# ExistentialRobotics/CORSAIR

Hardware: AMD Instinct MI355X
Metric: end-to-end queries/sec (embed+retrieve+register), Scan2CAD chair (higher is better)
Workload: dtype f32 sparse conv + embedding / f64 RANSAC, k-NN, Chamfer, top-k / f16 MFMA bounds and shortlists (survivors recounted in f64)

## Files before the change

corsair_amd/csrc/hardneg.hip:

```cpp
#include <hipcub/hipcub.hpp>

#include "nn_common.h"

namespace cs {

struct HnProb {
  int64_t t0;
  int32_t tn;
  int32_t pad;
};

struct HnTile {
  int32_t a0;
  int32_t an;
  int32_t prob;
  int32_t pad;
};

constexpr int HN_NG = 2;
constexpr int HN_QT = 4 * 32 * HN_NG;
constexpr int HN_KK = 4;
constexpr int32_t HN_NONE = 0x7fffffff;
constexpr int HN_EX_GRID = 4096;

// ... 47 lines not shown
}

__global__ void k_hn_pack_targets(const float* __restrict__ tf, int ld, const float* __restrict__ txyz,
                                  const int64_t* __restrict__ toff, _Float16* __restrict__ img,
                                  float4* __restrict__ t4, unsigned* __restrict__ seg_t2max_bits) {
  const int sg = blockIdx.y;
  const int64_t b = toff[sg], e = toff[sg + 1];
  float mx = 0.f;
  for (int64_t j = b + blockIdx.x * (int64_t)blockDim.x + threadIdx.x; j < e; j += (int64_t)gridDim.x * blockDim.x) {
    const double n2 = knf_pack_target_row(tf + j * ld, img + j * KNF_PITCH);
    t4[j] = make_float4(txyz[3 * j], txyz[3 * j + 1], txyz[3 * j + 2], (float)n2);
    mx = fmaxf(mx, (float)n2 * 1.0000002f);
  }
  knf_seg_max(mx, &seg_t2max_bits[sg]);
}

__global__ void k_hn_pack_anchors(const float* __restrict__ qf, int ld, const float* __restrict__ qxyz,
                                  const int32_t* __restrict__ anchor, const uint32_t* __restrict__ keys_sorted,
                                  const int32_t* __restrict__ vals_sorted, int64_t A, int n_prob,
                                  _Float16* __restrict__ qrows, float4* __restrict__ q4) {
  const int64_t i = blockIdx.x * (int64_t)blockDim.x + threadIdx.x;
  if (i >= A || keys_sorted[i] >= (uint32_t)n_prob) return;
  const int64_t r = anchor[vals_sorted[i]];
  knf_pack_query_row(qf + r * ld, qrows + i * 48);
  q4[i] = make_float4(qxyz[3 * r], qxyz[3 * r + 1], qxyz[3 * r + 2], 0.f);
}

__global__ __launch_bounds__(256) void k_hn_f16(const HnTile* __restrict__ tiles, const HnProb* __restrict__ probs,
                                                const _Float16* __restrict__ qrows, const float4* __restrict__ q4,
                                                const _Float16* __restrict__ img, const float4* __restrict__ t4,
                                                double r2, int use_excl, int32_t* __restrict__ cand_i,
                                                float* __restrict__ cand_tau) {
  constexpr int STAGE_BYTES = KNF_STAGE_BYTES;
  __shared__ __attribute__((aligned(1024))) char lds[2 * STAGE_BYTES];
  __shared__ __attribute__((aligned(16))) float tn_s[2][KNF_ROWS];
  __shared__ __attribute__((aligned(16))) float4 x_s[2][KNF_ROWS];
  const HnTile tile = tiles[blockIdx.x];
  if (tile.an == 0) return;
  const HnProb pb = probs[tile.prob];
  const int tid = threadIdx.x;
  const int lane = tid & 63;
  const int wave = __builtin_amdgcn_readfirstlane(tid >> 6);
  const int half = lane >> 5;
  const int col = lane & 31;
  f16x8 bop[HN_NG][3];
  double qx[HN_NG], qy[HN_NG], qz[HN_NG];
  bool qvalid[HN_NG];
  float bd[HN_NG][HN_KK], thr[HN_NG];
  int32_t bi[HN_NG][HN_KK];
#pragma unroll
  for (int g = 0; g < HN_NG; ++g) {
    const int qloc = wave * 32 * HN_NG + 32 * g + col;
    qvalid[g] = qloc < tile.an;
    const int64_t qpos = tile.a0 + (qvalid[g] ? qloc : 0);
    const _Float16* row = qrows + qpos * 48 + 8 * half;
#pragma unroll
    for (int m = 0; m < 3; ++m) bop[g][m] = *reinterpret_cast<const f16x8*>(row + 16 * m);
    const float4 p = q4[qpos];
    qx[g] = (double)p.x;
    qy[g] = (double)p.y;
    qz[g] = (double)p.z;
    thr[g] = INFINITY;
#pragma unroll
    for (int j = 0; j < HN_KK; ++j) {
      bd[g][j] = INFINITY;
      bi[g][j] = HN_NONE;
    }
  }
  const int t_hi = pb.tn;
  if (t_hi > 0) {
    const char* gimg = reinterpret_cast<const char*>(img + pb.t0 * KNF_PITCH) + lane * 16;
    const unsigned lds_base = __builtin_amdgcn_readfirstlane(lds_addr_of(lds));
    auto issue_dma = [&](int b, int base) { knf_issue_dma(gimg, lds_base, wave, b, base); };
    auto load_rows = [&](int base, float4& v) {
      int r = base + (tid % KNF_ROWS);
      r = r > t_hi - 1 ? t_hi - 1 : r;
      v = t4[pb.t0 + r];
    };
    auto store_rows = [&](int b, int base, const float4& v) {
      if (tid < KNF_ROWS) {
        tn_s[b][tid] = base + tid < t_hi ? v.w : INFINITY;
        x_s[b][tid] = v;
      }
    };
    {
      float4 v0;
      load_rows(0, v0);
      issue_dma(0, 0);
      store_rows(0, 0, v0);
    }
    int buf = 0;
    for (int base = 0; base < t_hi; base += KNF_ROWS) {
      asm volatile("s_waitcnt vmcnt(0)" ::: "memory");
      __syncthreads();
      const bool more = base + KNF_ROWS < t_hi;
      float4 v_next;
      load_rows(base + KNF_ROWS, v_next);
      if (more) issue_dma(buf ^ 1, base + KNF_ROWS);
#pragma unroll 1
      for (int t = 0; t < KNF_ROWS / 32; ++t) {
        if (base + 32 * t >= t_hi) break;
        f16x8 a[3];
        f32x16 c16;
        knf_load_tile(lds + buf * STAGE_BYTES, tn_s[buf], t, col, half, a, c16);
#pragma unroll
        for (int g = 0; g < HN_NG; ++g) {
          f32x16 d = __builtin_amdgcn_mfma_f32_32x32x16_f16(a[0], bop[g][0], c16, 0, 0, 0);
          d = knf_mfma_lo(a, bop[g], d);
#pragma unroll
          for (int r = 0; r < 16; ++r) {
            const bool hit = d[r] < thr[g];
            if (__any(hit)) {
              if (hit) {
                const int srow = knf_result_row(t, half, r);
                bool adm = true;
                if (use_excl) {
                  const float4 p = x_s[buf][srow];
                  const double dx = qx[g] - (double)p.x, dy = qy[g] - (double)p.y, dz = qz[g] - (double)p.z;
                  adm = !(((dx * dx + dy * dy) + dz * dz) < r2);
                }
                if (adm) knf_insert(bd[g], bi[g], d[r], base + srow);
              }
              thr[g] = fminf(thr[g], knf_pair_min(bd[g][HN_KK - 1]));
            }
          }
// ... 218 lines not shown
  while ((1LL << end_bit) <= (int64_t)n_prob) ++end_bit;
  size_t tmp_bytes = 0;
  CS_HIP_CHECK(hipcub::DeviceRadixSort::SortPairs(nullptr, tmp_bytes, keys.p, keys_sorted.p, vals.p, vals_sorted.p,
                                                  (int)A, 0, end_bit, s));
  CS_REQUIRE(tmp.alloc(tmp_bytes ? tmp_bytes : 1), CS_ERR_HIP, "cs_hardest_negatives: scratch allocation failed");
  CS_HIP_CHECK(hipcub::DeviceRadixSort::SortPairs(tmp.p, tmp_bytes, keys.p, keys_sorted.p, vals.p, vals_sorted.p, (int)A,
                                                  0, end_bit, s));

  if (!use_f16) {
    hipLaunchKernelGGL(k_hn_exhaustive, ex_grid, dim3(256), 0, s, d_qf, ld_q, d_qxyz, d_tf, ld_t, d_txyz, C,
                       d_anchor, keys_sorted.p, vals_sorted.p, A, n_prob, dprobs.p, r2, use_excl, (const int32_t*)nullptr,
                       d_idx, d_dist);
    CS_LAUNCH_CHECK();
    if (stats) {
      g_hn_stats[0] += (unsigned long long)A;
      g_hn_stats[1] += (unsigned long long)A;
    }
    return CS_OK;
  }

  const unsigned n_tile = (unsigned)(ceil_div(A, HN_QT) + n_prob);
  PoolBuf<HnTile> tiles((size_t)n_tile);
  PoolBuf<int32_t> pstart((size_t)n_prob + 1), cand((size_t)A * 2 * HN_KK), flag((size_t)A);
  PoolBuf<_Float16> qrows((size_t)A * 48), img((size_t)(nt_rows + KNF_ROWS) * KNF_PITCH);
  PoolBuf<float4> q4((size_t)A), t4((size_t)(nt_rows ? nt_rows : 1));
  PoolBuf<float> tau((size_t)A);
  PoolBuf<unsigned> t2max((size_t)ntseg);
  PoolBuf<int64_t> dtoff;
  CS_REQUIRE(tiles.p && pstart.p && cand.p && flag.p && qrows.p && img.p && q4.p && t4.p && tau.p && t2max.p, CS_ERR_HIP,
             "cs_hardest_negatives: scratch allocation failed");
  std::vector<int64_t> toff(h_toff, h_toff + ntseg + 1);
  rc = upload(dtoff, toff, s);
  if (rc) return rc;
  CS_HIP_CHECK(hipMemsetAsync(tiles.p, 0, sizeof(HnTile) * n_tile, s));
  CS_HIP_CHECK(hipMemsetAsync(t2max.p, 0, sizeof(unsigned) * ntseg, s));
  CS_HIP_CHECK(hipMemsetAsync(flag.p, 0, sizeof(int32_t) * (size_t)A, s));
  hipLaunchKernelGGL(k_hn_tiles, dim3(1), dim3(256), 0, s, keys_sorted.p, A, n_prob, pstart.p, tiles.p);
  CS_LAUNCH_CHECK();
  if (nt_rows) {
    hipLaunchKernelGGL(k_hn_pack_targets, dim3(16, (unsigned)ntseg), dim3(256), 0, s, d_tf, ld_t, d_txyz, dtoff.p, img.p,
                       t4.p, t2max.p);
    CS_LAUNCH_CHECK();
  }
  hipLaunchKernelGGL(k_hn_pack_anchors, dim3((unsigned)ceil_div(A, 256)), dim3(256), 0, s, d_qf, ld_q, d_qxyz, d_anchor,
                     keys_sorted.p, vals_sorted.p, A, n_prob, qrows.p, q4.p);
  CS_LAUNCH_CHECK();
  hipLaunchKernelGGL(k_hn_f16, dim3(n_tile), dim3(256), 0, s, tiles.p, dprobs.p, qrows.p, q4.p, img.p, t4.p, r2, use_excl,
// ... 21 lines not shown
```

corsair_amd/csrc/knn.hip:

```cpp
#include <hipcub/hipcub.hpp>


#include "nn_common.h"

namespace cs {

struct KnnWork {
  int64_t q0;
  int64_t t0;
  int64_t o0;
  int32_t qn;
  int32_t tn;
  int32_t prob;
  int32_t pad;
};

constexpr int KNN_MAXK = 8;
constexpr int KNN_TT = 128;

template <int DIM>
__global__ __launch_bounds__(256) void k_knn_feat(const KnnWork* __restrict__ work,
                                                  const float* __restrict__ qf,
                                                  const float* __restrict__ tf, int k,
                                                  const int32_t* __restrict__ qlabel,
// ... 68 lines not shown
    for (int j = 0; j < k; ++j) {
      double dj = INFINITY;
      int32_t ij = -1;
#pragma unroll
      for (int s = 0; s < KNN_MAXK; ++s)
        if (s == j) {
          dj = bd[s];
          ij = bi[s];
        }
      const int64_t orow = wk.o0 + tid;
      out_idx[orow * k + j] = ij;
      if (out_dist) out_dist[orow * k + j] = ij >= 0 ? sqrt(dj) : INFINITY;
    }
  }
}

constexpr int KNM_NG = 1;
constexpr int KNM_QT = 64 * KNM_NG;
constexpr int KNM_TT = 256;
constexpr int KNM_PITCH = 18;
constexpr int KNM_KK = 8;
constexpr int KNM_PEND = 4;

__global__ void k_seg_keys(const int64_t* __restrict__ off, int n_seg, const int32_t* __restrict__ label,
                           uint32_t* __restrict__ keys, int32_t* __restrict__ rows) {
  const int sg = blockIdx.y;
  const int64_t b = off[sg], e = off[sg + 1];
  for (int64_t i = b + blockIdx.x * (int64_t)blockDim.x + threadIdx.x; i < e; i += (int64_t)gridDim.x * blockDim.x) {
    const int l = label[i];
    keys[i] = (uint32_t)sg * 16u + (uint32_t)((l >= 0 && l < 8) ? l : 8);
    rows[i] = (int32_t)(i - b);
  }
}

__global__ void k_label_starts(const int64_t* __restrict__ off, int n_seg,
                               const uint32_t* __restrict__ keys_sorted, int32_t* __restrict__ lab_start) {
  const int i = blockIdx.x * blockDim.x + threadIdx.x;
  if (i >= n_seg * 10) return;
  const int sg = i / 10, l = i - sg * 10;
  const int64_t b = off[sg], e = off[sg + 1];
  const uint32_t key = (uint32_t)sg * 16u + (uint32_t)l;
  int64_t lo = b, hi = e;
  while (lo < hi) {
    const int64_t mid = (lo + hi) >> 1;
    if (keys_sorted[mid] < key) lo = mid + 1; else hi = mid;
  }
  lab_start[i] = (int32_t)(lo - b);
}

__global__ __launch_bounds__(256) void k_knn_mfma16(const KnnWork* __restrict__ work,
                                                    const float* __restrict__ qf,
                                                    const float* __restrict__ tf,
                                                    const double* __restrict__ qnorm,
                                                    const double* __restrict__ tnorm,
                                                    const int32_t* __restrict__ qlabel,
                                                    const int32_t* __restrict__ tlabel,
                                                    const int32_t* __restrict__ perm,
                                                    const int32_t* __restrict__ torder,
                                                    const int32_t* __restrict__ lab_start,
                                                    int32_t* __restrict__ cand_i) {
  __shared__ float t_lds[2][KNM_TT * KNM_PITCH];
  __shared__ double tn_lds[2][KNM_TT];
  __shared__ int32_t tl_lds[2][KNM_TT];
  __shared__ int32_t ti_lds[2][KNM_TT];
  __shared__ int32_t wrange[2][4];
  const KnnWork wk = work[blockIdx.x];
  const int tid = threadIdx.x;
  const int lane = tid & 63;
  const int wave = __builtin_amdgcn_readfirstlane(tid >> 6);
  const int col = lane & 15;
// ... 246 lines not shown
constexpr int KNF_QT = 4 * 32 * KNF_NG;
static_assert(KNF_QT == 256, "tiles of the f16 path and of the exhaustive fallback must coincide");
constexpr int KNF_KK = 8;
constexpr int KNF_PEND = 4;

__global__ void k_knf_pack_targets(const float* __restrict__ tf, const int64_t* __restrict__ toff, int n_seg,
                                   const int32_t* __restrict__ torder, _Float16* __restrict__ img,
                                   float* __restrict__ tn32, int32_t* __restrict__ ti32,
                                   unsigned* __restrict__ seg_t2max_bits) {
  const int sg = blockIdx.y;
  const int64_t b = toff[sg], e = toff[sg + 1];
  float mx = 0.f;
  for (int64_t j = b + blockIdx.x * (int64_t)blockDim.x + threadIdx.x; j < e; j += (int64_t)gridDim.x * blockDim.x) {
    const int32_t loc = torder ? torder[j] : (int32_t)(j - b);
    const double n2 = knf_pack_target_row(tf + (b + loc) * 16, img + j * KNF_PITCH);
    tn32[j] = (float)n2;
    ti32[j] = loc;
    mx = fmaxf(mx, (float)n2 * 1.0000002f);
  }
  knf_seg_max(mx, &seg_t2max_bits[sg]);
}

__global__ void k_knf_pack_queries(const float* __restrict__ qf, int64_t n, _Float16* __restrict__ qrows,
                                   float* __restrict__ qn32) {
  const int64_t i = blockIdx.x * (int64_t)blockDim.x + threadIdx.x;
  if (i >= n) return;
  const double n2 = knf_pack_query_row(qf + i * 16, qrows + i * 48);
  qn32[i] = (float)n2 * 1.0000002f;
}

template <int PASS>
__global__ __launch_bounds__(256) void k_knn_f16(const KnnWork* __restrict__ work,
                                                 const _Float16* __restrict__ qrows,
                                                 const _Float16* __restrict__ img,
                                                 const float* __restrict__ tn32,
                                                 const int32_t* __restrict__ ti32,
                                                 const int32_t* __restrict__ qlabel,
                                                 const int32_t* __restrict__ perm,
                                                 const int32_t* __restrict__ lab_start,
                                                 int32_t* __restrict__ cand_i, float* __restrict__ cand_tau,
                                                 float* __restrict__ thr0, const float* __restrict__ qn32,
                                                 const unsigned* __restrict__ seg_t2max_bits, int kq) {
  constexpr int STAGE_BYTES = KNF_STAGE_BYTES;
  __shared__ __attribute__((aligned(1024))) char lds[2 * STAGE_BYTES];
  __shared__ __attribute__((aligned(16))) float tn_s[2][KNF_ROWS];
  __shared__ int32_t wrange[2][4];
  const KnnWork wk = work[blockIdx.x];
  const int tid = threadIdx.x;
  const int lane = tid & 63;
  const int wave = __builtin_amdgcn_readfirstlane(tid >> 6);
  const int half = lane >> 5;
  const int col = lane & 31;
  const bool use_labels = qlabel != nullptr;
  f16x8 bop[KNF_NG][3];
  int want[KNF_NG];
  bool qvalid[KNF_NG];
  int wmin = 0x7fffffff, wmax = -2;
#pragma unroll
  for (int g = 0; g < KNF_NG; ++g) {
    const int qloc = wave * 32 * KNF_NG + 32 * g + col;
    qvalid[g] = qloc < wk.qn;
    const int64_t qrow = wk.q0 + (qvalid[g] ? qloc : 0);
    const _Float16* row = qrows + qrow * 48 + 8 * half;
#pragma unroll
    for (int m = 0; m < 3; ++m) bop[g][m] = *reinterpret_cast<const f16x8*>(row + 16 * m);
    want[g] = -1;
    if (use_labels) {
      const int ql = qlabel[qrow];
      want[g] = (qvalid[g] && ql >= 0 && ql < 8) ? perm[wk.prob * 8 + ql] : -2;
      if (want[g] >= 0) wmin = min(wmin, want[g]);
      wmax = max(wmax, want[g]);
    }
  }
  int lab_lo = -1, lab_hi = -1;
  if (use_labels) {
#pragma unroll
    for (int off = 32; off >= 1; off >>= 1) {
      wmin = min(wmin, __shfl_xor(wmin, off));
      wmax = max(wmax, __shfl_xor(wmax, off));
    }
    if (lane == 0) {
      wrange[0][wave] = wmin;
      wrange[1][wave] = wmax;
    }
    __syncthreads();
    lab_lo = min(min(wrange[0][0], wrange[0][1]), min(wrange[0][2], wrange[0][3]));
    lab_hi = max(max(wrange[1][0], wrange[1][1]), max(wrange[1][2], wrange[1][3]));
    if (lab_hi > 7) lab_hi = 7;
// ... 47 lines not shown
    if (t_hi <= t_lo) continue;
    float thr_eff[KNF_NG];
#pragma unroll
    for (int g = 0; g < KNF_NG; ++g) thr_eff[g] = (!use_labels || want[g] == lab) ? thr[g] : -INFINITY;
    auto issue_dma = [&](int b, int base) { knf_issue_dma(gimg, lds_base, wave, b, base); };
    auto load_rows = [&](int base, float& tn) {
      int r = base + (tid % KNF_ROWS);
      r = r > t_hi - 1 ? t_hi - 1 : r;
      r = r < t_lo ? t_lo : r;
      tn = tn32[wk.t0 + r];
    };
    auto store_rows = [&](int b, int base, float tn) {
      if (tid < KNF_ROWS) tn_s[b][tid] = base + tid < t_hi ? tn : INFINITY;
    };
    __syncthreads();
    {
      float tn0;
      load_rows(t_lo, tn0);
      issue_dma(0, t_lo);
      store_rows(0, t_lo, tn0);
    }
    int buf = 0;
    for (int base = t_lo; base < t_hi; base += KNF_ROWS) {
      asm volatile("s_waitcnt vmcnt(0)" ::: "memory");
      __syncthreads();
      const bool more = base + KNF_ROWS < t_hi;
      float tn_next;
      load_rows(base + KNF_ROWS, tn_next);
      if (more) issue_dma(buf ^ 1, base + KNF_ROWS);
#pragma unroll 1
      for (int t = 0; t < KNF_ROWS / 32; ++t) {
        if (base + 32 * t >= t_hi) break;
        f16x8 a[3];
        f32x16 c16;
        knf_load_tile(lds + buf * STAGE_BYTES, tn_s[buf], t, col, half, a, c16);
#pragma unroll
        for (int g = 0; g < KNF_NG; ++g) {
          f32x16 d = __builtin_amdgcn_mfma_f32_32x32x16_f16(a[0], bop[g][0], c16, 0, 0, 0);
          if (PASS == 1) {
            float m = fminf(fminf(d[0], d[1]), d[2]);
            m = fminf(fminf(m, d[3]), d[4]);
            m = fminf(fminf(m, d[5]), d[6]);
            m = fminf(fminf(m, d[7]), d[8]);
            m = fminf(fminf(m, d[9]), d[10]);
            m = fminf(fminf(m, d[11]), d[12]);
            m = fminf(fminf(m, d[13]), d[14]);
            m = fminf(m, d[15]);
            if (use_labels && want[g] != lab) m = INFINITY;
            const float o0 = tb[g][0], o1 = tb[g][1], o2 = tb[g][2], o3 = tb[g][3], o4 = tb[g][4], o5 = tb[g][5];
            tb[g][0] = fminf(o0, m);
            tb[g][1] = __builtin_amdgcn_fmed3f(o0, o1, m);
            tb[g][2] = __builtin_amdgcn_fmed3f(o1, o2, m);
            tb[g][3] = __builtin_amdgcn_fmed3f(o2, o3, m);
            tb[g][4] = __builtin_amdgcn_fmed3f(o3, o4, m);
            tb[g][5] = __builtin_amdgcn_fmed3f(o4, o5, m);
            continue;
// ... 5 lines not shown
            const bool hit = d[r] < thr_eff[g] - 1.0e30f;
#else
            const bool hit = d[r] < thr_eff[g];
#endif
            if (__any(hit)) {
              if (hit) {
#pragma unroll
                for (int e = KNF_PEND - 1; e > 0; --e) {
                  pd[g][e] = pd[g][e - 1];
                  pi[g][e] = pi[g][e - 1];
                }
                pd[g][0] = d[r];
                pi[g][0] = base + knf_result_row(t, half, r);
                ++pn[g];
              }
              if (__any(pn[g] == KNF_PEND)) {
                rank_pending(g);
                thr_eff[g] = (!use_labels || want[g] == lab) ? thr[g] : -INFINITY;
              }
            }
          }
        }
      }
      if (more) store_rows(buf ^ 1, base + KNF_ROWS, tn_next);
      buf ^= 1;
    }
  }
  if (PASS == 1) {
#pragma unroll
    for (int g = 0; g < KNF_NG; ++g) {
      float bk = INFINITY;
#pragma unroll
      for (int j = 0; j < 6; ++j)
        if (j == kq - 1) bk = tb[g][j];
      bk = fminf(bk, __shfl_xor(bk, 32));
      const int qloc = wave * 32 * KNF_NG + 32 * g + col;
      if (qvalid[g] && half == 0) {
        const float budget = qn32[wk.q0 + qloc] + __uint_as_float(seg_t2max_bits[wk.pad]);
        thr0[wk.o0 + qloc] = bk + budget * (0x1.0p-9f + 0x1.0p-14f) + fabsf(bk) * 0x1.0p-20f;
      }
    }
    return;
  }
#pragma unroll
  for (int g = 0; g < KNF_NG; ++g) {
    rank_pending(g);
    const int qloc = wave * 32 * KNF_NG + 32 * g + col;
    if (qvalid[g]) {
      const int64_t base = ((wk.o0 + qloc) * 2 + half) * KNF_KK;
// ... 87 lines not shown
  int64_t i = blockIdx.x * (int64_t)blockDim.x + threadIdx.x;
  unsigned long long v = (i < n && flag[i]) ? 1ULL : 0ULL;
#pragma unroll
  for (int off = 32; off >= 1; off >>= 1) v += __shfl_xor(v, off);
  if ((threadIdx.x & 63) == 0 && v) atomicAdd(out, v);
}

int cs::count_flagged(const int32_t* d_flag, int64_t n, unsigned long long* host_out, hipStream_t s,
                      const char* who) {
  PoolBuf<unsigned long long> cnt(1);
  CS_REQUIRE(cnt.p, CS_ERR_HIP, "%s: scratch allocation failed", who);
  CS_HIP_CHECK(hipMemsetAsync(cnt.p, 0, sizeof(unsigned long long), s));
  hipLaunchKernelGGL(k_count_flags, dim3((unsigned)ceil_div(n, 256)), dim3(256), 0, s, d_flag, n, cnt.p);
  CS_HIP_CHECK(hipMemcpyAsync(host_out, cnt.p, sizeof(*host_out), hipMemcpyDeviceToHost, s));
  CS_HIP_CHECK(hipStreamSynchronize(s));
  return CS_OK;
}

struct KnnOptions {
  enum Path { F16, F64, EXHAUSTIVE };
  Path path;
  bool two_pass;
  bool stats;
};
static KnnOptions read_options() {
  const char* mfma = getenv("CS_KNN_MFMA");
  KnnOptions o;
  o.path = KnnOptions::F16;
  if (mfma && mfma[0] == '0') o.path = KnnOptions::EXHAUSTIVE;
  if (mfma && mfma[0] == '6') o.path = KnnOptions::F64;
  o.two_pass = !env_first_is("CS_KNN_TWOPASS", '0');
  o.stats = env_first_is("CS_KNN_STATS", '1');
  return o;
}

struct KnnCall {
  const float *d_qf, *d_tf;
  const int64_t *h_qoff, *h_toff;
  int nqseg, ntseg;
  int dim, k;
  const int32_t *d_qlabel, *d_tlabel, *d_perm;
  int32_t* d_idx;
  double* d_dist;
  const KnnWork* d_work;
  unsigned n_work;
  int64_t out_row;
  double flop;
  hipStream_t s;
};

static int label_order(const int32_t* d_tlabel, const int64_t* d_toff, int ntseg, int64_t nt_rows, hipStream_t s,
                       PoolBuf<int32_t>& torder, PoolBuf<int32_t>& lab_start) {
  PoolBuf<int32_t> rows_in;
  PoolBuf<uint32_t> keys, keys_sorted;
  PoolBuf<char> tmp;
  CS_REQUIRE(torder.alloc((size_t)nt_rows) && keys.alloc((size_t)nt_rows) && keys_sorted.alloc((size_t)nt_rows) &&
                 rows_in.alloc((size_t)nt_rows) && lab_start.alloc((size_t)ntseg * 10),
             CS_ERR_HIP, "cs_knn_feat: scratch allocation failed");
  hipLaunchKernelGGL(k_seg_keys, dim3(16, (unsigned)ntseg), dim3(256), 0, s, d_toff, ntseg, d_tlabel, keys.p,
                     rows_in.p);
  int end_bit = 4;
  while ((1LL << end_bit) < (int64_t)ntseg * 16) ++end_bit;
  size_t tmp_bytes = 0;
  CS_HIP_CHECK(hipcub::DeviceRadixSort::SortPairs(nullptr, tmp_bytes, keys.p, keys_sorted.p, rows_in.p, torder.p,
                                                  (int)nt_rows, 0, end_bit, s));
  CS_REQUIRE(tmp.alloc(tmp_bytes ? tmp_bytes : 1), CS_ERR_HIP, "cs_knn_feat: scratch allocation failed");
  CS_HIP_CHECK(hipcub::DeviceRadixSort::SortPairs(tmp.p, tmp_bytes, keys.p, keys_sorted.p, rows_in.p, torder.p,
                                                  (int)nt_rows, 0, end_bit, s));
  hipLaunchKernelGGL(k_label_starts, dim3((unsigned)ceil_div((int64_t)ntseg * 10, 256)), dim3(256), 0, s, d_toff,
                     ntseg, keys_sorted.p, lab_start.p);
  return CS_OK;
}

static int knn_f16(const KnnCall& c, const KnnOptions& opt) {
  hipStream_t s = c.s;
  const int64_t nq_rows = c.h_qoff[c.nqseg], nt_rows = c.h_toff[c.ntseg], out_row = c.out_row;
  const int ntseg = c.ntseg;
  CS_REQUIRE(nt_rows < (1LL << 31) && ntseg < (1 << 27), CS_ERR_UNSUPPORTED,
             "cs_knn_feat: too many target rows / segments");
  PoolBuf<_Float16> qrows((size_t)(nq_rows ? nq_rows : 1) * 48);
  PoolBuf<_Float16> img((size_t)(nt_rows + KNF_ROWS) * KNF_PITCH);
  PoolBuf<float> tn32((size_t)(nt_rows ? nt_rows : 1)), tau((size_t)(out_row ? out_row : 1));
  PoolBuf<int32_t> ti32((size_t)(nt_rows ? nt_rows : 1)), cand((size_t)(out_row ? out_row : 1) * 2 * KNF_KK);
  PoolBuf<int32_t> qflag((size_t)(out_row ? out_row : 1)), tile_flag(c.n_work);
  PoolBuf<unsigned> t2max((size_t)ntseg);
  const bool two_pass = c.k <= 6 && opt.two_pass;
  PoolBuf<float> thr0((size_t)(out_row ? out_row : 1)), qn32((size_t)(nq_rows ? nq_rows : 1));
  PoolBuf<int32_t> torder, lab_start;
  PoolBuf<int64_t> dtoff;
  CS_REQUIRE(qrows.p && img.p && tn32.p && tau.p && ti32.p && cand.p && qflag.p && tile_flag.p && t2max.p && thr0.p &&
                 qn32.p,
             CS_ERR_HIP, "cs_knn_feat: scratch allocation failed");
  std::vector<int64_t> toff(c.h_toff, c.h_toff + ntseg + 1);
  int rc = upload(dtoff, toff, s);
  if (rc) return rc;
  const bool labelled = c.d_tlabel && nt_rows;
  if (labelled) {
    rc = label_order(c.d_tlabel, dtoff.p, ntseg, nt_rows, s, torder, lab_start);
    if (rc) return rc;
  }
  CS_HIP_CHECK(hipMemsetAsync(t2max.p, 0, sizeof(unsigned) * ntseg, s));
  CS_HIP_CHECK(hipMemsetAsync(tile_flag.p, 0, sizeof(int32_t) * c.n_work, s));
  if (nt_rows)
    hipLaunchKernelGGL(k_knf_pack_targets, dim3(16, (unsigned)ntseg), dim3(256), 0, s, c.d_tf, dtoff.p, ntseg,
                       labelled ? torder.p : (const int32_t*)nullptr, img.p, tn32.p, ti32.p, t2max.p);
  if (nq_rows)
    hipLaunchKernelGGL(k_knf_pack_queries, dim3((unsigned)ceil_div(nq_rows, 256)), dim3(256), 0, s, c.d_qf, nq_rows,
                       qrows.p, qn32.p);
  {
    ProfScope prof("knn", s, c.flop);
    const dim3 grid(c.n_work);
    const int32_t* labs = labelled ? lab_start.p : (const int32_t*)nullptr;
    if (two_pass)
      hipLaunchKernelGGL(k_knn_f16<1>, grid, dim3(256), 0, s, c.d_work, qrows.p, img.p, tn32.p, ti32.p, c.d_qlabel,
                         c.d_perm, labs, cand.p, tau.p, thr0.p, qn32.p, t2max.p, c.k);
    hipLaunchKernelGGL(k_knn_f16<0>, grid, dim3(256), 0, s, c.d_work, qrows.p, img.p, tn32.p, ti32.p, c.d_qlabel,
                       c.d_perm, labs, cand.p, tau.p, two_pass ? thr0.p : (float*)nullptr, qn32.p, t2max.p, c.k);
    hipLaunchKernelGGL(k_knn_rescore_f16, grid, dim3(256), 0, s, c.d_work, c.d_qf, c.d_tf, cand.p, tau.p, t2max.p,
                       c.k, c.d_idx, c.d_dist, qflag.p, tile_flag.p);
    hipLaunchKernelGGL((k_knn_feat<16>), grid, dim3(256), 0, s, c.d_work, c.d_qf, c.d_tf, c.k, c.d_qlabel,
                       c.d_tlabel, c.d_perm, c.d_idx, c.d_dist, tile_flag.p, qflag.p);
    CS_LAUNCH_CHECK();
  }
  if (opt.stats && out_row > 0) {
    unsigned long long h = 0;
    rc = count_flagged(qflag.p, out_row, &h, s, "cs_knn_feat");
    if (rc) return rc;
    g_knn_stats[0] += (unsigned long long)out_row;
    g_knn_stats[1] += h;
  }
  return CS_OK;
}

static int knn_f64(const KnnCall& c) {
  hipStream_t s = c.s;
  const int64_t nq_rows = c.h_qoff[c.nqseg], nt_rows = c.h_toff[c.ntseg], out_row = c.out_row;
  const int ntseg = c.ntseg;
  CS_REQUIRE(nt_rows < (1LL << 31) && ntseg < (1 << 27), CS_ERR_UNSUPPORTED,
             "cs_knn_feat: too many target rows / segments");
  PoolBuf<double> qnorm((size_t)(nq_rows ? nq_rows : 1)), tnorm((size_t)(nt_rows ? nt_rows : 1));
  PoolBuf<int32_t> cand((size_t)(out_row ? out_row : 1) * 4 * KNM_KK);
  PoolBuf<int32_t> torder, lab_start;
  PoolBuf<int64_t> dtoff;
  CS_REQUIRE(qnorm.p && tnorm.p && cand.p, CS_ERR_HIP, "cs_knn_feat: scratch allocation failed");
  if (nq_rows) row_norms(c.d_qf, nq_rows, 16, qnorm.p, s);
// ... 9 lines not shown
                     c.d_qlabel, c.d_tlabel, c.d_perm, c.d_tlabel ? torder.p : nullptr,
                     c.d_tlabel ? lab_start.p : nullptr, cand.p);
  hipLaunchKernelGGL(k_knn_rescore16, dim3(c.n_work), dim3(KNM_QT), 0, s, c.d_work, c.d_qf, c.d_tf, cand.p, c.k,
                     c.d_idx, c.d_dist);
  CS_LAUNCH_CHECK();
  return CS_OK;
}

static int knn_exhaustive(const KnnCall& c) {
  ProfScope prof("knn", c.s, c.flop);
  const dim3 grid(c.n_work);
  const int32_t* none = nullptr;
  if (c.dim == 16)
    hipLaunchKernelGGL((k_knn_feat<16>), grid, dim3(256), 0, c.s, c.d_work, c.d_qf, c.d_tf, c.k, c.d_qlabel,
                       c.d_tlabel, c.d_perm, c.d_idx, c.d_dist, none, none);
  else if (c.dim == 32)
    hipLaunchKernelGGL((k_knn_feat<32>), grid, dim3(256), 0, c.s, c.d_work, c.d_qf, c.d_tf, c.k, c.d_qlabel,
                       c.d_tlabel, c.d_perm, c.d_idx, c.d_dist, none, none);
  else
    hipLaunchKernelGGL((k_knn_feat<3>), grid, dim3(256), 0, c.s, c.d_work, c.d_qf, c.d_tf, c.k, c.d_qlabel,
                       c.d_tlabel, c.d_perm, c.d_idx, c.d_dist, none, none);
  CS_LAUNCH_CHECK();
  return CS_OK;
}

extern "C" {

void cs_knn_shortlist_stats(uint64_t out[2], int reset) { read_stats(g_knn_stats, out, reset); }

int cs_knn_feat(const float* d_qf, const int64_t* h_qoff, const float* d_tf,
                const int64_t* h_toff, const int32_t* h_qseg, const int32_t* h_tseg, int n_prob,
                int dim, int k, const int32_t* d_qlabel, const int32_t* d_tlabel,
                const int32_t* d_perm, int32_t* d_idx, double* d_dist, void* stream) {
  CS_REQUIRE(d_qf && d_tf && h_qoff && h_toff && h_qseg && h_tseg && d_idx, CS_ERR_INVALID,
             "cs_knn_feat: NULL argument");
  CS_REQUIRE(k >= 1 && k <= KNN_MAXK, CS_ERR_UNSUPPORTED, "cs_knn_feat: k = %d not in [1, %d]", k,
             KNN_MAXK);
  CS_REQUIRE(dim == 16 || dim == 32 || dim == 3, CS_ERR_UNSUPPORTED,
             "cs_knn_feat: feature dimension %d not supported (3, 16, 32)", dim);
  CS_REQUIRE((d_qlabel == nullptr) == (d_tlabel == nullptr) &&
                 (d_qlabel == nullptr) == (d_perm == nullptr),
             CS_ERR_INVALID, "cs_knn_feat: labels and perm must be given together");
  if (n_prob <= 0) return CS_OK;
  hipStream_t s = (hipStream_t)stream;
  pool_use_stream(s);
  const KnnOptions opt = read_options();
// ... 5 lines not shown
  for (int p = 0; p < n_prob; ++p) {
    CS_REQUIRE(h_qseg[p] >= 0 && h_tseg[p] >= 0, CS_ERR_INVALID,
               "cs_knn_feat: negative segment id in problem %d", p);
    nqseg = h_qseg[p] + 1 > nqseg ? h_qseg[p] + 1 : nqseg;
    ntseg = h_tseg[p] + 1 > ntseg ? h_tseg[p] + 1 : ntseg;
    const int64_t q0 = h_qoff[h_qseg[p]], t0 = h_toff[h_tseg[p]];
    int64_t qn = h_qoff[h_qseg[p] + 1] - q0, tn = h_toff[h_tseg[p] + 1] - t0;
    CS_REQUIRE(qn >= 0 && tn >= 0 && tn < (1LL << 31), CS_ERR_INVALID,
               "cs_knn_feat: bad segment in problem %d", p);
    for (int64_t q = 0; q < qn; q += qtile) {
      KnnWork w;
      w.q0 = q0 + q;
      w.t0 = t0;
      w.o0 = out_row + q;
      w.qn = (int32_t)(qn - q < qtile ? qn - q : qtile);
      w.tn = (int32_t)tn;
      w.prob = p;
      w.pad = h_tseg[p];
      work.push_back(w);
    }
    out_row += qn;
  }
  if (work.empty()) return CS_OK;
  PoolBuf<KnnWork> dwork;
  const int rc = upload(dwork, work, s);
  if (rc) return rc;
  double knn_flop = 0.0;
  for (const KnnWork& w : work) knn_flop += 3.0 * (double)w.qn * (double)w.tn * (double)dim;
  const KnnCall call = {d_qf, d_tf, h_qoff, h_toff, nqseg, ntseg, dim, k, d_qlabel, d_tlabel, d_perm, d_idx, d_dist,
                        dwork.p, (unsigned)work.size(), out_row, knn_flop, s};
  if (path == KnnOptions::F16) return knn_f16(call, opt);
  if (path == KnnOptions::F64) return knn_f64(call);
  return knn_exhaustive(call);
}

}
```

corsair_amd/csrc/nn_common.h:

```cpp
#pragma once
#include <stdlib.h>

#include <atomic>
#include <vector>

#include "common.h"

namespace cs {

using f64x4 = __attribute__((ext_vector_type(4))) double;
using f16x8 = __attribute__((ext_vector_type(8))) _Float16;
using f32x16 = __attribute__((ext_vector_type(16))) float;

__device__ __forceinline__ void knf_split(float v, _Float16* hi, _Float16* lo) {
  const _Float16 h = (_Float16)v;
  *hi = h;
  *lo = (_Float16)(v - (float)h);
}

constexpr int KNF_PITCH = 56;
constexpr int KNF_ROWS = 192;
constexpr int KNF_STAGE_BYTES = KNF_ROWS * KNF_PITCH * 2;
constexpr int KNF_STAGE_KIB = KNF_STAGE_BYTES / 1024;
static_assert(KNF_STAGE_BYTES % 1024 == 0, "a stage is copied in 1-KiB pieces");
constexpr double KNF_EPS_REL = 0x1.0p-15;
constexpr double KNF_RANGE = 1.0e8;

__device__ __forceinline__ double knf_pack_target_row(const float* __restrict__ f, _Float16* __restrict__ dst) {
  union {
    _Float16 h[KNF_PITCH];
    uint4 v[7];
  } row;
  double n2 = 0.0;
#pragma unroll
  for (int c = 0; c < 16; ++c) {
    _Float16 hi, lo;
    knf_split(f[c], &hi, &lo);
    row.h[c] = hi;
    row.h[16 + c] = lo;
    row.h[32 + c] = hi;
    n2 = fma((double)f[c], (double)f[c], n2);
  }
#pragma unroll
  for (int c = 48; c < KNF_PITCH; ++c) row.h[c] = (_Float16)0.0f;
  uint4* d4 = reinterpret_cast<uint4*>(dst);
#pragma unroll
  for (int c = 0; c < 7; ++c) d4[c] = row.v[c];
  return n2;
}

__device__ __forceinline__ double knf_pack_query_row(const float* __restrict__ f, _Float16* __restrict__ dst) {
  union {
    _Float16 h[48];
    uint4 v[6];
  } row;
  double n2 = 0.0;
#pragma unroll
  for (int c = 0; c < 16; ++c) {
    _Float16 hi, lo;
    knf_split(-2.0f * f[c], &hi, &lo);
    row.h[c] = hi;
    row.h[16 + c] = hi;
    row.h[32 + c] = lo;
    n2 = fma((double)f[c], (double)f[c], n2);
  }
  uint4* d4 = reinterpret_cast<uint4*>(dst);
#pragma unroll
  for (int c = 0; c < 6; ++c) d4[c] = row.v[c];
  return n2;
}

__device__ __forceinline__ void knf_seg_max(float mx, unsigned* __restrict__ seg_bits) {
#pragma unroll
  for (int off = 32; off >= 1; off >>= 1) mx = fmaxf(mx, __shfl_xor(mx, off));
  if ((threadIdx.x & 63) == 0 && mx > 0.f) atomicMax(seg_bits, __float_as_uint(mx));
}

__device__ __forceinline__ void knf_issue_dma(const char* gimg, unsigned lds_base, int wave, int b, int base) {
  const char* gp = gimg + (int64_t)base * (KNF_PITCH * 2);
#pragma unroll
  for (int i = 0; i < (KNF_STAGE_KIB + 3) / 4; ++i) {
    const int piece = wave + 4 * i;
    if (piece < KNF_STAGE_KIB) lds_dma16(gp + piece * 1024, lds_base + b * KNF_STAGE_BYTES + piece * 1024);
  }
}

__device__ __forceinline__ void knf_load_tile(const char* stage, const float* tn, int t, int col, int half,
                                              f16x8 (&a)[3], f32x16& c16) {
  const _Float16* arow = reinterpret_cast<const _Float16*>(stage) + (t * 32 + col) * KNF_PITCH + 8 * half;
#pragma unroll
  for (int m = 0; m < 3; ++m) a[m] = *reinterpret_cast<const f16x8*>(arow + 16 * m);
#pragma unroll
  for (int q4 = 0; q4 < 4; ++q4) {
    const float4 v = *reinterpret_cast<const float4*>(&tn[t * 32 + 8 * q4 + 4 * half]);
    c16[4 * q4 + 0] = v.x; c16[4 * q4 + 1] = v.y; c16[4 * q4 + 2] = v.z; c16[4 * q4 + 3] = v.w;
  }
}
__device__ __forceinline__ int knf_result_row(int t, int half, int r) { return t * 32 + 4 * half + (r & 3) + 8 * (r >> 2); }

__device__ __forceinline__ f32x16 knf_mfma_lo(const f16x8 (&a)[3], const f16x8 (&b)[3], f32x16 d) {
  d = __builtin_amdgcn_mfma_f32_32x32x16_f16(a[1], b[1], d, 0, 0, 0);
  return __builtin_amdgcn_mfma_f32_32x32x16_f16(a[2], b[2], d, 0, 0, 0);
}

template <int KK>
__device__ __forceinline__ void knf_insert(float (&bd)[KK], int32_t (&bi)[KK], float cd, int32_t ci) {
  bool carry = false;
#pragma unroll
  for (int s2 = 0; s2 < KK; ++s2) {
    if (carry || cd < bd[s2]) {
      carry = true;
      const float td = bd[s2];
      const int32_t ti = bi[s2];
      bd[s2] = cd;
      bi[s2] = ci;
      cd = td;
      ci = ti;
    }
  }
}
__device__ __forceinline__ float knf_pair_min(float t) { return fminf(t, __shfl_xor(t, 32)); }

__device__ __forceinline__ double knf_chain16(const double (&q)[16], const float* __restrict__ tp) {
  double d = 0.0;
#pragma unroll
// ... 40 lines not shown
```

Baseline: 1949.

## Shrink f16 split rows, replace label radix sort, and deal kNN work across XCDs

The split-f16 target and query rows drop their duplicated hi copy. Target pitch goes from 56 to 40 halves and query rows from 48 to 32, so the MFMA terms reuse the hi/lo pieces by swapping operands. This cuts the LDS stage size and global traffic. The hipcub radix sort used for label ordering is replaced by a single per-segment ballot-based counting kernel. Memsets are folded into the query-pack kernel, work items are reordered on the host to balance cost across the 8 XCDs, and an optional s_memtime trace instrumentation path is added.

```diff
diff --git a/corsair_amd/csrc/hardneg.hip b/corsair_amd/csrc/hardneg.hip
--- a/corsair_amd/csrc/hardneg.hip
+++ b/corsair_amd/csrc/hardneg.hip
@@ -93,7 +93,7 @@
   const int64_t i = blockIdx.x * (int64_t)blockDim.x + threadIdx.x;
   if (i >= A || keys_sorted[i] >= (uint32_t)n_prob) return;
   const int64_t r = anchor[vals_sorted[i]];
-  knf_pack_query_row(qf + r * ld, qrows + i * 48);
+  knf_pack_query_row(qf + r * ld, qrows + i * KNF_QROW);
   q4[i] = make_float4(qxyz[3 * r], qxyz[3 * r + 1], qxyz[3 * r + 2], 0.f);
 }
 
@@ -114,7 +114,7 @@
   const int wave = __builtin_amdgcn_readfirstlane(tid >> 6);
   const int half = lane >> 5;
   const int col = lane & 31;
-  f16x8 bop[HN_NG][3];
+  f16x8 bop[HN_NG][2];
   double qx[HN_NG], qy[HN_NG], qz[HN_NG];
   bool qvalid[HN_NG];
   float bd[HN_NG][HN_KK], thr[HN_NG];
@@ -124,9 +124,9 @@
     const int qloc = wave * 32 * HN_NG + 32 * g + col;
     qvalid[g] = qloc < tile.an;
     const int64_t qpos = tile.a0 + (qvalid[g] ? qloc : 0);
-    const _Float16* row = qrows + qpos * 48 + 8 * half;
-#pragma unroll
-    for (int m = 0; m < 3; ++m) bop[g][m] = *reinterpret_cast<const f16x8*>(row + 16 * m);
+    const _Float16* row = qrows + qpos * KNF_QROW + 8 * half;
+#pragma unroll
+    for (int m = 0; m < 2; ++m) bop[g][m] = *reinterpret_cast<const f16x8*>(row + 16 * m);
     const float4 p = q4[qpos];
     qx[g] = (double)p.x;
     qy[g] = (double)p.y;
@@ -171,7 +171,7 @@
 #pragma unroll 1
       for (int t = 0; t < KNF_ROWS / 32; ++t) {
         if (base + 32 * t >= t_hi) break;
-        f16x8 a[3];
+        f16x8 a[2];
         f32x16 c16;
         knf_load_tile(lds + buf * STAGE_BYTES, tn_s[buf], t, col, half, a, c16);
 #pragma unroll
@@ -436,7 +436,7 @@
   const unsigned n_tile = (unsigned)(ceil_div(A, HN_QT) + n_prob);
   PoolBuf<HnTile> tiles((size_t)n_tile);
   PoolBuf<int32_t> pstart((size_t)n_prob + 1), cand((size_t)A * 2 * HN_KK), flag((size_t)A);
-  PoolBuf<_Float16> qrows((size_t)A * 48), img((size_t)(nt_rows + KNF_ROWS) * KNF_PITCH);
+  PoolBuf<_Float16> qrows((size_t)A * KNF_QROW), img((size_t)(nt_rows + KNF_ROWS) * KNF_PITCH);
   PoolBuf<float4> q4((size_t)A), t4((size_t)(nt_rows ? nt_rows : 1));
   PoolBuf<float> tau((size_t)A);
   PoolBuf<unsigned> t2max((size_t)ntseg);
diff --git a/corsair_amd/csrc/knn.hip b/corsair_amd/csrc/knn.hip
--- a/corsair_amd/csrc/knn.hip
+++ b/corsair_amd/csrc/knn.hip
@@ -1,5 +1,5 @@
-#include <hipcub/hipcub.hpp>
-
+#include <algorithm>
+#include <numeric>
 
 #include "nn_common.h"
 
@@ -114,30 +114,54 @@
 constexpr int KNM_KK = 8;
 constexpr int KNM_PEND = 4;
 
-__global__ void k_seg_keys(const int64_t* __restrict__ off, int n_seg, const int32_t* __restrict__ label,
-                           uint32_t* __restrict__ keys, int32_t* __restrict__ rows) {
-  const int sg = blockIdx.y;
-  const int64_t b = off[sg], e = off[sg + 1];
-  for (int64_t i = b + blockIdx.x * (int64_t)blockDim.x + threadIdx.x; i < e; i += (int64_t)gridDim.x * blockDim.x) {
-    const int l = label[i];
-    keys[i] = (uint32_t)sg * 16u + (uint32_t)((l >= 0 && l < 8) ? l : 8);
-    rows[i] = (int32_t)(i - b);
-  }
-}
-
-__global__ void k_label_starts(const int64_t* __restrict__ off, int n_seg,
-                               const uint32_t* __restrict__ keys_sorted, int32_t* __restrict__ lab_start) {
-  const int i = blockIdx.x * blockDim.x + threadIdx.x;
-  if (i >= n_seg * 10) return;
-  const int sg = i / 10, l = i - sg * 10;
-  const int64_t b = off[sg], e = off[sg + 1];
-  const uint32_t key = (uint32_t)sg * 16u + (uint32_t)l;
-  int64_t lo = b, hi = e;
-  while (lo < hi) {
-    const int64_t mid = (lo + hi) >> 1;
-    if (keys_sorted[mid] < key) lo = mid + 1; else hi = mid;
-  }
-  lab_start[i] = (int32_t)(lo - b);
+constexpr int LBO_WAVES = 16;
+__global__ __launch_bounds__(64 * LBO_WAVES) void k_label_order(const int32_t* __restrict__ label,
+                                                                const int64_t* __restrict__ off,
+                                                                int32_t* __restrict__ torder,
+                                                                int32_t* __restrict__ lab_start) {
+  __shared__ int wcnt[LBO_WAVES][9];
+  const int sg = blockIdx.x;
+  const int64_t r0 = off[sg];
+  const int n = (int)(off[sg + 1] - r0);
+  const int lane = threadIdx.x & 63, wave = threadIdx.x >> 6;
+  const int chunk = ((n + LBO_WAVES - 1) / LBO_WAVES + 63) / 64 * 64;
+  const int64_t c0l = (int64_t)wave * chunk;
+  const int c0 = (int)(c0l < n ? c0l : n), c1 = (int)(c0l + chunk < n ? c0l + chunk : n);
+  auto class_of = [&](int64_t r) {
+    if (r >= c1) return -1;
+    const int l = label[r0 + r];
+    return (l >= 0 && l < 8) ? l : 8;
+  };
+  int cnt = 0;
+  for (int rb = c0; rb < c1; rb += 64) {
+    const int l = class_of((int64_t)rb + lane);
+#pragma unroll
+    for (int q = 0; q < 9; ++q) {
+      const unsigned long long m = __ballot(l == q);
+      if (lane == q) cnt += __popcll(m);
+    }
+  }
+  if (lane < 9) wcnt[wave][lane] = cnt;
+  __syncthreads();
+  int run = 0;
+  if (lane < 10) {
+    for (int q = 0; q < 9; ++q)
+      for (int w = 0; w < LBO_WAVES; ++w)
+        if (q < lane || (q == lane && w < wave)) run += wcnt[w][q];
+    if (wave == 0) lab_start[sg * 10 + lane] = run;
+  }
+  for (int rb = c0; rb < c1; rb += 64) {
+    const int l = class_of((int64_t)rb + lane);
+    int pos = 0;
+#pragma unroll
+    for (int q = 0; q < 9; ++q) {
+      const unsigned long long m = __ballot(l == q);
+      const int first = __shfl(run, q);
+      if (l == q) pos = first + __popcll(m & ((1ULL << lane) - 1ULL));
+      if (lane == q) run += __popcll(m);
+    }
+    if (l >= 0) torder[r0 + pos] = rb + lane;
+  }
 }
 
 __global__ __launch_bounds__(256) void k_knn_mfma16(const KnnWork* __restrict__ work,
@@ -430,14 +454,18 @@
 }
 
 __global__ void k_knf_pack_queries(const float* __restrict__ qf, int64_t n, _Float16* __restrict__ qrows,
-                                   float* __restrict__ qn32) {
+                                   float* __restrict__ qn32, unsigned* __restrict__ seg_t2max_bits, int n_seg,
+                                   int32_t* __restrict__ tile_flag, int n_tile) {
   const int64_t i = blockIdx.x * (int64_t)blockDim.x + threadIdx.x;
+  const int64_t stride = gridDim.x * (int64_t)blockDim.x;
+  for (int64_t j = i; j < n_seg; j += stride) seg_t2max_bits[j] = 0u;
+  for (int64_t j = i; j < n_tile; j += stride) tile_flag[j] = 0;
   if (i >= n) return;
-  const double n2 = knf_pack_query_row(qf + i * 16, qrows + i * 48);
+  const double n2 = knf_pack_query_row(qf + i * 16, qrows + i * KNF_QROW);
   qn32[i] = (float)n2 * 1.0000002f;
 }
 
-template <int PASS>
+template <int PASS, bool TRACE>
 __global__ __launch_bounds__(256) void k_knn_f16(const KnnWork* __restrict__ work,
                                                  const _Float16* __restrict__ qrows,
                                                  const _Float16* __restrict__ img,
@@ -448,8 +476,11 @@
                                                  const int32_t* __restrict__ lab_start,
                                                  int32_t* __restrict__ cand_i, float* __restrict__ cand_tau,
                                                  float* __restrict__ thr0, const float* __restrict__ qn32,
-                                                 const unsigned* __restrict__ seg_t2max_bits, int kq) {
+                                                 const unsigned* __restrict__ seg_t2max_bits, int kq,
+                                                 unsigned long long* __restrict__ trace) {
   constexpr int STAGE_BYTES = KNF_STAGE_BYTES;
+  unsigned long long t_start = 0, t_vm = 0, t_bar = 0, t_tile = 0, n_stage = 0, ta = 0, tb0 = 0, tc = 0;
+  if (TRACE) t_start = __builtin_amdgcn_s_memtime();
   __shared__ __attribute__((aligned(1024))) char lds[2 * STAGE_BYTES];
   __shared__ __attribute__((aligned(16))) float tn_s[2][KNF_ROWS];
   __shared__ int32_t wrange[2][4];
@@ -460,7 +491,7 @@
   const int half = lane >> 5;
   const int col = lane & 31;
   const bool use_labels = qlabel != nullptr;
-  f16x8 bop[KNF_NG][3];
+  f16x8 bop[KNF_NG][2];
   int want[KNF_NG];
   bool qvalid[KNF_NG];
   int wmin = 0x7fffffff, wmax = -2;
@@ -469,9 +500,9 @@
     const int qloc = wave * 32 * KNF_NG + 32 * g + col;
     qvalid[g] = qloc < wk.qn;
     const int64_t qrow = wk.q0 + (qvalid[g] ? qloc : 0);
-    const _Float16* row = qrows + qrow * 48 + 8 * half;
-#pragma unroll
-    for (int m = 0; m < 3; ++m) bop[g][m] = *reinterpret_cast<const f16x8*>(row + 16 * m);
+    const _Float16* row = qrows + qrow * KNF_QROW + 8 * half;
+#pragma unroll
+    for (int m = 0; m < 2; ++m) bop[g][m] = *reinterpret_cast<const f16x8*>(row + 16 * m);
     want[g] = -1;
     if (use_labels) {
       const int ql = qlabel[qrow];
@@ -565,16 +596,25 @@
     }
     int buf = 0;
     for (int base = t_lo; base < t_hi; base += KNF_ROWS) {
+      if (TRACE) ta = __builtin_amdgcn_s_memtime();
       asm volatile("s_waitcnt vmcnt(0)" ::: "memory");
+      if (TRACE) tb0 = __builtin_amdgcn_s_memtime();
       __syncthreads();
+      if (TRACE) {
+        tc = __builtin_amdgcn_s_memtime();
+        t_vm += tb0 - ta;
+        t_bar += tc - tb0;
+        ++n_stage;
+      }
       const bool more = base + KNF_ROWS < t_hi;
       float tn_next;
       load_rows(base + KNF_ROWS, tn_next);
       if (more) issue_dma(buf ^ 1, base + KNF_ROWS);
+      if (TRACE) tc = __builtin_amdgcn_s_memtime();
 #pragma unroll 1
       for (int t = 0; t < KNF_ROWS / 32; ++t) {
         if (base + 32 * t >= t_hi) break;
-        f16x8 a[3];
+        f16x8 a[2];
         f32x16 c16;
         knf_load_tile(lds + buf * STAGE_BYTES, tn_s[buf], t, col, half, a, c16);
 #pragma unroll
@@ -626,9 +666,18 @@
           }
         }
       }
+      if (TRACE) t_tile += __builtin_amdgcn_s_memtime() - tc;
       if (more) store_rows(buf ^ 1, base + KNF_ROWS, tn_next);
       buf ^= 1;
     }
+  }
+  if (TRACE && lane == 0) {
+    atomicAdd(&trace[0], t_vm);
+    atomicAdd(&trace[1], t_bar);
+    atomicAdd(&trace[2], t_tile);
+    atomicAdd(&trace[3], (unsigned long long)__builtin_amdgcn_s_memtime() - t_start);
+    atomicAdd(&trace[4], n_stage);
+    atomicAdd(&trace[5], 1ULL);
   }
   if (PASS == 1) {
 #pragma unroll
@@ -762,6 +811,8 @@
   Path path;
   bool two_pass;
   bool stats;
+  bool xcd_deal;
+  bool trace;
 };
 static KnnOptions read_options() {
   const char* mfma = getenv("CS_KNN_MFMA");
@@ -771,6 +822,8 @@
   if (mfma && mfma[0] == '6') o.path = KnnOptions::F64;
   o.two_pass = !env_first_is("CS_KNN_TWOPASS", '0');
   o.stats = env_first_is("CS_KNN_STATS", '1');
+  o.xcd_deal = !env_first_is("CS_KNN_XCD", '0');
+  o.trace = env_first_is("CS_KNN_TRACE", '1');
   return o;
 }
 
@@ -791,24 +844,27 @@
 
 static int label_order(const int32_t* d_tlabel, const int64_t* d_toff, int ntseg, int64_t nt_rows, hipStream_t s,
                        PoolBuf<int32_t>& torder, PoolBuf<int32_t>& lab_start) {
-  PoolBuf<int32_t> rows_in;
-  PoolBuf<uint32_t> keys, keys_sorted;
-  PoolBuf<char> tmp;
-  CS_REQUIRE(torder.alloc((size_t)nt_rows) && keys.alloc((size_t)nt_rows) && keys_sorted.alloc((size_t)nt_rows) &&
-                 rows_in.alloc((size_t)nt_rows) && lab_start.alloc((size_t)ntseg * 10),
-             CS_ERR_HIP, "cs_knn_feat: scratch allocation failed");
-  hipLaunchKernelGGL(k_seg_keys, dim3(16, (unsigned)ntseg), dim3(256), 0, s, d_toff, ntseg, d_tlabel, keys.p,
-                     rows_in.p);
-  int end_bit = 4;
-  while ((1LL << end_bit) < (int64_t)ntseg * 16) ++end_bit;
-  size_t tmp_bytes = 0;
-  CS_HIP_CHECK(hipcub::DeviceRadixSort::SortPairs(nullptr, tmp_bytes, keys.p, keys_sorted.p, rows_in.p, torder.p,
-                                                  (int)nt_rows, 0, end_bit, s));
-  CS_REQUIRE(tmp.alloc(tmp_bytes ? tmp_bytes : 1), CS_ERR_HIP, "cs_knn_feat: scratch allocation failed");
-  CS_HIP_CHECK(hipcub::DeviceRadixSort::SortPairs(tmp.p, tmp_bytes, keys.p, keys_sorted.p, rows_in.p, torder.p,
-                                                  (int)nt_rows, 0, end_bit, s));
-  hipLaunchKernelGGL(k_label_starts, dim3((unsigned)ceil_div((int64_t)ntseg * 10, 256)), dim3(256), 0, s, d_toff,
-                     ntseg, keys_sorted.p, lab_start.p);
+  CS_REQUIRE(torder.alloc((size_t)nt_rows) && lab_start.alloc((size_t)ntseg * 10), CS_ERR_HIP,
+             "cs_knn_feat: scratch allocation failed");
+  hipLaunchKernelGGL(k_label_order, dim3((unsigned)ntseg), dim3(64 * LBO_WAVES), 0, s, d_tlabel, d_toff, torder.p,
+                     lab_start.p);
+  return CS_OK;
+}
+
+static int knn_trace_report(const unsigned long long* d_trace, unsigned n_work, hipStream_t s) {
+  unsigned long long h[16];
+  CS_HIP_CHECK(hipMemcpyAsync(h, d_trace, sizeof(h), hipMemcpyDeviceToHost, s));
+  CS_HIP_CHECK(hipStreamSynchronize(s));
+  for (int pass = 1; pass >= 0; --pass) {
+    const unsigned long long* t = h + 8 * pass;
+    if (!t[5]) continue;
+    const double life = (double)t[3], nw = (double)t[5], ns = (double)(t[4] ? t[4] : 1);
+    fprintf(stderr, "[knn trace] %s pass: %u workgroups, %.0f waves, %.1f stages per wave; per wave %.0f cyc = vmcnt "
+            "%.0f (%.3f) + barrier %.0f (%.3f) + tiles %.0f (%.3f) + rest %.0f; per stage: vmcnt %.0f barrier %.0f "
+            "tiles %.0f\n", pass ? "threshold" : "shortlist", n_work, nw, ns / nw, life / nw, t[0] / nw, t[0] / life,
+            t[1] / nw, t[1] / life, t[2] / nw, t[2] / life, (life - t[0] - t[1] - t[2]) / nw, t[0] / ns, t[1] / ns,
+            t[2] / ns);
+  }
   return CS_OK;
 }
 
@@ -818,7 +874,7 @@
   const int ntseg = c.ntseg;
   CS_REQUIRE(nt_rows < (1LL << 31) && ntseg < (1 << 27), CS_ERR_UNSUPPORTED,
              "cs_knn_feat: too many target rows / segments");
-  PoolBuf<_Float16> qrows((size_t)(nq_rows ? nq_rows : 1) * 48);
+  PoolBuf<_Float16> qrows((size_t)(nq_rows ? nq_rows : 1) * KNF_QROW);
   PoolBuf<_Float16> img((size_t)(nt_rows + KNF_ROWS) * KNF_PITCH);
   PoolBuf<float> tn32((size_t)(nt_rows ? nt_rows : 1)), tau((size_t)(out_row ? out_row : 1));
   PoolBuf<int32_t> ti32((size_t)(nt_rows ? nt_rows : 1)), cand((size_t)(out_row ? out_row : 1) * 2 * KNF_KK);
@@ -834,33 +890,44 @@
   std::vector<int64_t> toff(c.h_toff, c.h_toff + ntseg + 1);
   int rc = upload(dtoff, toff, s);
   if (rc) return rc;
+  PoolBuf<unsigned long long> trace;
+  if (opt.trace) {
+    CS_REQUIRE(trace.alloc(16), CS_ERR_HIP, "cs_knn_feat: scratch allocation failed");
+    CS_HIP_CHECK(hipMemsetAsync(trace.p, 0, 16 * sizeof(unsigned long long), s));
+  }
   const bool labelled = c.d_tlabel && nt_rows;
   if (labelled) {
     rc = label_order(c.d_tlabel, dtoff.p, ntseg, nt_rows, s, torder, lab_start);
     if (rc) return rc;
   }
-  CS_HIP_CHECK(hipMemsetAsync(t2max.p, 0, sizeof(unsigned) * ntseg, s));
-  CS_HIP_CHECK(hipMemsetAsync(tile_flag.p, 0, sizeof(int32_t) * c.n_work, s));
+  hipLaunchKernelGGL(k_knf_pack_queries, dim3((unsigned)ceil_div(nq_rows ? nq_rows : 1, 256)), dim3(256), 0, s, c.d_qf, nq_rows,
+                     qrows.p, qn32.p, t2max.p, ntseg, tile_flag.p, (int)c.n_work);
   if (nt_rows)
     hipLaunchKernelGGL(k_knf_pack_targets, dim3(16, (unsigned)ntseg), dim3(256), 0, s, c.d_tf, dtoff.p, ntseg,
                        labelled ? torder.p : (const int32_t*)nullptr, img.p, tn32.p, ti32.p, t2max.p);
-  if (nq_rows)
-    hipLaunchKernelGGL(k_knf_pack_queries, dim3((unsigned)ceil_div(nq_rows, 256)), dim3(256), 0, s, c.d_qf, nq_rows,
-                       qrows.p, qn32.p);
   {
     ProfScope prof("knn", s, c.flop);
     const dim3 grid(c.n_work);
     const int32_t* labs = labelled ? lab_start.p : (const int32_t*)nullptr;
+    unsigned long long* const tr = trace.p;
+    float* const thr_in = two_pass ? thr0.p : (float*)nullptr;
+    auto* const pass1 = tr ? k_knn_f16<1, true> : k_knn_f16<1, false>;
+    auto* const pass0 = tr ? k_knn_f16<0, true> : k_knn_f16<0, false>;
     if (two_pass)
-      hipLaunchKernelGGL(k_knn_f16<1>, grid, dim3(256), 0, s, c.d_work, qrows.p, img.p, tn32.p, ti32.p, c.d_qlabel,
-                         c.d_perm, labs, cand.p, tau.p, thr0.p, qn32.p, t2max.p, c.k);
-    hipLaunchKernelGGL(k_knn_f16<0>, grid, dim3(256), 0, s, c.d_work, qrows.p, img.p, tn32.p, ti32.p, c.d_qlabel,
-                       c.d_perm, labs, cand.p, tau.p, two_pass ? thr0.p : (float*)nullptr, qn32.p, t2max.p, c.k);
+      hipLaunchKernelGGL(pass1, grid, dim3(256), 0, s, c.d_work, qrows.p, img.p,
+                         tn32.p, ti32.p, c.d_qlabel, c.d_perm, labs, cand.p, tau.p, thr0.p, qn32.p, t2max.p, c.k,
+                         tr ? tr + 8 : tr);
+    hipLaunchKernelGGL(pass0, grid, dim3(256), 0, s, c.d_work, qrows.p, img.p,
+                       tn32.p, ti32.p, c.d_qlabel, c.d_perm, labs, cand.p, tau.p, thr_in, qn32.p, t2max.p, c.k, tr);
     hipLaunchKernelGGL(k_knn_rescore_f16, grid, dim3(256), 0, s, c.d_work, c.d_qf, c.d_tf, cand.p, tau.p, t2max.p,
                        c.k, c.d_idx, c.d_dist, qflag.p, tile_flag.p);
     hipLaunchKernelGGL((k_knn_feat<16>), grid, dim3(256), 0, s, c.d_work, c.d_qf, c.d_tf, c.k, c.d_qlabel,
                        c.d_tlabel, c.d_perm, c.d_idx, c.d_dist, tile_flag.p, qflag.p);
     CS_LAUNCH_CHECK();
+  }
+  if (trace.p) {
+    rc = knn_trace_report(trace.p, c.n_work, s);
+    if (rc) return rc;
   }
   if (opt.stats && out_row > 0) {
     unsigned long long h = 0;
@@ -916,6 +983,42 @@
                        c.d_tlabel, c.d_perm, c.d_idx, c.d_dist, none, none);
   CS_LAUNCH_CHECK();
   return CS_OK;
+}
+
+static void deal_by_xcd(std::vector<KnnWork>& work) {
+  const size_t n = work.size();
+  if (n <= 8) return;
+  std::vector<uint32_t> ord(n);
+  std::iota(ord.begin(), ord.end(), 0u);
+  std::stable_sort(ord.begin(), ord.end(), [&](uint32_t a, uint32_t b) {
+    return work[a].tn != work[b].tn ? work[a].tn > work[b].tn : work[a].pad < work[b].pad;
+  });
+  auto cost = [&](uint32_t i) { return (double)work[i].tn + 256.0; };
+  double total = 0.0;
+  for (uint32_t i : ord) total += cost(i);
+  size_t head[8], tail[8];
+  {
+    double run = 0.0;
+    size_t i = 0;
+    for (int x = 0; x < 8; ++x) {
+      head[x] = i;
+      const double upto = total * (double)(x + 1) / 8.0;
+      while (i < n && (x == 7 || run + 0.5 * cost(ord[i]) < upto)) run += cost(ord[i++]);
+      tail[x] = i;
+    }
+  }
+  std::vector<KnnWork> dealt(n);
+  for (size_t b = 0; b < n; ++b) {
+    int x = (int)(b & 7);
+    if (head[x] < tail[x]) {
+      dealt[b] = work[ord[head[x]++]];
+      continue;
+    }
+    for (int y = 0; y < 8; ++y)
+      if (tail[y] - head[y] > tail[x] - head[x]) x = y;
+    dealt[b] = work[ord[--tail[x]]];
+  }
+  work.swap(dealt);
 }
 
 extern "C" {
@@ -967,6 +1070,7 @@
     out_row += qn;
   }
   if (work.empty()) return CS_OK;
+  if (opt.xcd_deal) deal_by_xcd(work);
   PoolBuf<KnnWork> dwork;
   const int rc = upload(dwork, work, s);
   if (rc) return rc;
diff --git a/corsair_amd/csrc/nn_common.h b/corsair_amd/csrc/nn_common.h
--- a/corsair_amd/csrc/nn_common.h
+++ b/corsair_amd/csrc/nn_common.h
@@ -18,7 +18,8 @@
   *lo = (_Float16)(v - (float)h);
 }
 
-constexpr int KNF_PITCH = 56;
+constexpr int KNF_PITCH = 40;
+constexpr int KNF_QROW = 32;
 constexpr int KNF_ROWS = 192;
 constexpr int KNF_STAGE_BYTES = KNF_ROWS * KNF_PITCH * 2;
 constexpr int KNF_STAGE_KIB = KNF_STAGE_BYTES / 1024;
@@ -29,7 +30,7 @@
 __device__ __forceinline__ double knf_pack_target_row(const float* __restrict__ f, _Float16* __restrict__ dst) {
   union {
     _Float16 h[KNF_PITCH];
-    uint4 v[7];
+    uint4 v[KNF_PITCH / 8];
   } row;
   double n2 = 0.0;
 #pragma unroll
@@ -38,21 +39,20 @@
     knf_split(f[c], &hi, &lo);
     row.h[c] = hi;
     row.h[16 + c] = lo;
-    row.h[32 + c] = hi;
     n2 = fma((double)f[c], (double)f[c], n2);
   }
 #pragma unroll
-  for (int c = 48; c < KNF_PITCH; ++c) row.h[c] = (_Float16)0.0f;
+  for (int c = 32; c < KNF_PITCH; ++c) row.h[c] = (_Float16)0.0f;
   uint4* d4 = reinterpret_cast<uint4*>(dst);
 #pragma unroll
-  for (int c = 0; c < 7; ++c) d4[c] = row.v[c];
+  for (int c = 0; c < KNF_PITCH / 8; ++c) d4[c] = row.v[c];
   return n2;
 }
 
 __device__ __forceinline__ double knf_pack_query_row(const float* __restrict__ f, _Float16* __restrict__ dst) {
   union {
-    _Float16 h[48];
-    uint4 v[6];
+    _Float16 h[KNF_QROW];
+    uint4 v[KNF_QROW / 8];
   } row;
   double n2 = 0.0;
 #pragma unroll
@@ -60,13 +60,12 @@
     _Float16 hi, lo;
     knf_split(-2.0f * f[c], &hi, &lo);
     row.h[c] = hi;
-    row.h[16 + c] = hi;
-    row.h[32 + c] = lo;
+    row.h[16 + c] = lo;
     n2 = fma((double)f[c], (double)f[c], n2);
   }
   uint4* d4 = reinterpret_cast<uint4*>(dst);
 #pragma unroll
-  for (int c = 0; c < 6; ++c) d4[c] = row.v[c];
+  for (int c = 0; c < KNF_QROW / 8; ++c) d4[c] = row.v[c];
   return n2;
 }
 
@@ -86,10 +85,10 @@
 }
 
 __device__ __forceinline__ void knf_load_tile(const char* stage, const float* tn, int t, int col, int half,
-                                              f16x8 (&a)[3], f32x16& c16) {
+                                              f16x8 (&a)[2], f32x16& c16) {
   const _Float16* arow = reinterpret_cast<const _Float16*>(stage) + (t * 32 + col) * KNF_PITCH + 8 * half;
 #pragma unroll
-  for (int m = 0; m < 3; ++m) a[m] = *reinterpret_cast<const f16x8*>(arow + 16 * m);
+  for (int m = 0; m < 2; ++m) a[m] = *reinterpret_cast<const f16x8*>(arow + 16 * m);
 #pragma unroll
   for (int q4 = 0; q4 < 4; ++q4) {
     const float4 v = *reinterpret_cast<const float4*>(&tn[t * 32 + 8 * q4 + 4 * half]);
@@ -98,9 +97,9 @@
 }
 __device__ __forceinline__ int knf_result_row(int t, int half, int r) { return t * 32 + 4 * half + (r & 3) + 8 * (r >> 2); }
 
-__device__ __forceinline__ f32x16 knf_mfma_lo(const f16x8 (&a)[3], const f16x8 (&b)[3], f32x16 d) {
-  d = __builtin_amdgcn_mfma_f32_32x32x16_f16(a[1], b[1], d, 0, 0, 0);
-  return __builtin_amdgcn_mfma_f32_32x32x16_f16(a[2], b[2], d, 0, 0, 0);
+__device__ __forceinline__ f32x16 knf_mfma_lo(const f16x8 (&a)[2], const f16x8 (&b)[2], f32x16 d) {
+  d = __builtin_amdgcn_mfma_f32_32x32x16_f16(a[1], b[0], d, 0, 0, 0);
+  return __builtin_amdgcn_mfma_f32_32x32x16_f16(a[0], b[1], d, 0, 0, 0);
 }
 
 template <int KK>
```

After: 1957 (median of 3 runs). No clear change (+0.4%).
